# pvjosue/CWFA

Measured on AMD Instinct MI355X. Metric: volumes/sec inverse-pass @512×512×96 fp32; NLL match vs ref (1/2/4/8 GPU), higher is better.
Workload: dtype f32 (storage, accumulation, wavelets, couplings); convolution products on the bf16 matrix cores from an exact three-way bf16 split of both fp32 operands, six products per fp32 product: fp32-equivalent; plain-fp32-MFMA figure: fp32_mfma; 1 GPU; 512x512x96 volume, 4-scale CWFA (CAT blocks, 64 ch) + LRNN inverse, z=0, batch 1/GPU, random-init weights (BASELINE.json configs[2]); precision=split, parallelism=replicated x1 (independent volumes per GPU, no collective)

## Files before the change

cwfa_amd/_lib.py:

```python
import ctypes as C
import os

_HERE = os.path.dirname(os.path.abspath(__file__))
LIB_PATH = os.path.join(_HERE, "libcwfa_hip.so")

CLAMP = {"NONE": 0, "ATAN": 1, "TANH": 2, "SIGMOID": 3}
ACT = {None: 0, "none": 0, "elu": 1, "prelu": 2, "gelu": 3, "relu": 4}
CHAIN_MAX = 8

c_f32p = C.c_void_p
c_i64p = C.c_void_p
c_f64p = C.c_void_p


class AffineStage(C.Structure):
    _fields_ = [("s_raw", c_f32p), ("t", c_f32p), ("s_bs", C.c_int64), ("t_bs", C.c_int64), ("clamp_kind", C.c_int),
                ("clamp", C.c_float), ("pre_scale", C.c_float), ("t_neg_div_sqrt2", C.c_int), ("perm", c_i64p),
                ("perm_axis", C.c_int), ("gin", C.c_int)]


class Chain(C.Structure):
    _fields_ = [("n_stages", C.c_int), ("stage", AffineStage * CHAIN_MAX), ("src_c", C.c_void_p), ("src_h", C.c_void_p)]


# ... 53 lines not shown
    "cwfa_haar2d_inv_f32": (i, [p, p, i, i, i, i, i, f, p]),
    "cwfa_haar3d_fwd_f32": (i, [p, p, i, i, i, i, i, f, i64, p]),
    "cwfa_haar3d_inv_f32": (i, [p, p, i, i, i, i, i, f, i64, p]),
    "cwfa_gather_f32": (i, [p, p, p, i, i, i, i, i, i64, i64, p]),
    "cwfa_affine_f32": (i, [p, p, C.POINTER(AffineStage), i, i, i, i, i, i64, i64, p, p, p]),
    "cwfa_channel_affine_f32": (i, [p, p, p, p, i, p, p, i, i, i64, i64, i64, p]),
    "cwfa_chain_inv_f32": (i, [p, p, p, C.POINTER(Chain), i, i, i, i, i64, i64, i64, p, p]),
    "cwfa_chain_fwd_f32": (i, [p, p, p, C.POINTER(Chain), p, i, i, i, i, i64, i64, i64, p, p, p]),
    "cwfa_conv2d_packed_floats": (i64, [i, i, i]),
    "cwfa_conv2d_pack_f32": (i, [p, p, i, i, i, i, p]),
    "cwfa_conv2d_f32": (i, [p, p, p, i, i, i, i, i, i, i64, i64, C.POINTER(ConvOpts), p]),
    "cwfa_subnet_pack1x1_f32": (i, [p, p, p]),
    "cwfa_subnet_layer_tape_f32": (i, [p, p, p, p, p, p, p, i, i, i, i64, i64, i64, p]),
    "cwfa_subnet_layer_f32": (i, [p, p, p, p, p, p, i, i, i, i64, i64, p]),
    "cwfa_conv3d_1k1_f32": (i, [p, p, p, p, p, p, p, i, i, i, i, i, p]),
    "cwfa_conv3d_1k1_split_f32": (i, [p, p, p, p, p, p, p, i, i, i, i, i, p]),
    "cwfa_channel_stats_f32": (i, [p, p, i, i, i64, i64, p]),
    "cwfa_bn_fold_f32": (i, [p, d, p, p, p, p, f, p, i, p, p, i, p]),
    "cwfa_maxpool_f32": (i, [p, p, p, p, p, i, i, i, i, i, i, p]),
    "cwfa_sample_stats_f32": (i, [p, p, i, i64, p]),
    "cwfa_layernorm_apply_f32": (i, [p, p, p, p, f, p, i, i64, p]),
    "cwfa_attention_combine_f32": (i, [p, p, p, p, p, p, p, p, i, i, i64, p]),
    "cwfa_scale_channels_f32": (i, [p, p, p, i, i, i64, p]),
    "cwfa_axpby_f32": (i, [p, p, f, f, p, i64, p]),
    "cwfa_bn_running_update_f32": (i, [p, C.c_double, f, p, p, p, i, p]),
    "cwfa_bn_finish_f32": (i, [p, d, p, p, p, f, i, p, p, f, p, p, f, f, i, p, p, i, i, p]),
    "cwfa_chain_bwd_f32": (i, [p, p, C.POINTER(Chain), C.POINTER(ChainGrads), p, p, i, i, i, i, i64, i64, i64, f, f, i, p, p]),
    "cwfa_affine_bwd_f32": (i, [p, p, C.POINTER(AffineStage), i, i, i, i, i, i64, i64, p, p, p, p, p]),
    "cwfa_chain_inv_bwd_f32": (i, [p, p, C.POINTER(Chain), C.POINTER(ChainGrads), i, i, i, i, i64, i64, f, i, i, p, p, p, p]),
    "cwfa_conv2d_wgrad_workspace_bytes": (i64, [i, i, i, i, i, i]),
    "cwfa_conv2d_wgrad_f32": (i, [p, p, p, p, p, i, i, i, i, i, i, i64, i64, f, p]),
    "cwfa_elu_bwd_f32": (i, [p, p, p, p, i, i64, i64, i64, i64, i64, p]),
    "cwfa_conv3d_hidden_fwd_f32": (i, [p, p, p, p, i, i, i, i, i, p]),
    "cwfa_conv3d_hidden_bwd_f32": (i, [p, p, p, p, p, p, i, i, i, i, i, p]),
    "cwfa_conv3d_input_bwd_f32": (i, [p, p, p, i, i, i, i, i, p]),
    "cwfa_conv3d_wgrad_workspace_bytes": (i64, [i, i, i, i]),
    "cwfa_conv3d_wgrad_f32": (i, [p, p, p, p, p, i, i, i, i, i, i, i, f, p]),
    "cwfa_prelu_bwd_f32": (i, [p, p, p, p, p, i, i64, i64, i64, i64, p]),
    "cwfa_plane_affine_f32": (i, [p, p, p, i, p, p, i, i, i64, i64, i64, i64, p]),
    "cwfa_bn_bwd_stats_f32": (i, [p, p, p, p, i, i, i64, i64, i64, p]),
    "cwfa_bn_act_bwd_f32": (i, [p, p, p, i, p, p, p, p, p, i, i, i64, i64, i64, i64, p]),
    "cwfa_maxpool2_bwd_f32": (i, [p, p, p, p, i, i, i, i, p]),
    "cwfa_gelu_f32": (i, [p, p, p, i64, i, p]),
    "cwfa_layernorm_bwd_f32": (i, [p, p, p, p, p, p, p, p, p, i, i64, p]),
    "cwfa_attention_bwd_f32": (i, [p, p, p, p, p, p, p, p, p, i, i, i64, p]),
    "cwfa_split_workspace_bytes": (i64, [i, i, i64]),
    "cwfa_split_input_f32": (i, [p, p, i, i, i64, i64, p, p, i64, p, i64, p]),
    "cwfa_conv_split_packed_bytes": (i64, [i, i, i]),
    "cwfa_conv_split_pack_f32": (i, [p, p, i, i, i, i, p]),
    "cwfa_conv_split_f32": (i, [p, p, p, i, i, i, i, i, i, i64, C.POINTER(ConvOpts), p]),
    "cwfa_conv3x3_split_packed_bytes": (i64, [i, i]),
    "cwfa_conv3x3_split_pack_f32": (i, [p, p, i, i, p]),
    "cwfa_conv3x3_split_f32": (i, [p, p, p, i, i, i, i, i, i64, i64, C.POINTER(ConvOpts), p]),
    "cwfa_conv7x7_split_packed_bytes": (i64, [i, i]),
    "cwfa_conv7x7_split_pack_f32": (i, [p, p, i, i, p]),
    "cwfa_conv7x7_split_f32": (i, [p, p, p, i, i, i, i, i, i64, i64, C.POINTER(ConvOpts), p]),
    "cwfa_couple_rows": (i, [i, p]),
    "cwfa_conv3x3_split_couple_f32": (i, [p, p, p, i, i, i, i, i64, C.POINTER(Couple), p]),
    "cwfa_subnet_layer_split_packed_bytes": (i64, []),
    "cwfa_subnet_layer_split_pack_f32": (i, [p, p, p, p]),
    "cwfa_subnet_layer_split_f32": (i, [p, p, p, p, p, i, i, i, i64, i64, i, p]),
    "cwfa_subnet_layer_split_tape_f32": (i, [p, p, p, p, p, p, i, i, i, i64, i64, i64, p]),
    "cwfa_subnet_layer_first_packed_bytes": (i64, []),
    "cwfa_subnet_layer_first_pack_f32": (i, [p, p, p, i, p, p]),
    "cwfa_subnet_layer_first_f32": (i, [p, p, p, p, p, p, i, i, i, i, i64, i64, i64, i, p]),
    "cwfa_extract_views_f32": (i, [p, p, p, i, i, i, i, i, i, f, f, i64, p]),
    "cwfa_eval_splits": (i64, [i, i64]),
    "cwfa_volume_extrema_f32": (i, [p, p, p, p, i, i64, i64, i64, C.POINTER(EvalAffine), p]),
    "cwfa_volume_metrics_f32": (i, [p, p, p, p, i, i64, i64, i64, C.POINTER(EvalAffine), f, f, f, p]),
    "cwfa_mip3_f32": (i, [p, p, p, p, p, p, i, i, i, i, i64, i64, i, C.POINTER(EvalAffine), C.POINTER(EvalPost), p]),
    "cwfa_projection_compose_f32": (i, [p, p, p, p, p, i, i, i, i, i, i, i, p]),
    "cwfa_roi_means_f32": (i, [p, p, p, i, i, i, i, i, i64, p]),
    "cwfa_select_positive_f32": (i, [p, i, i64, i64, i64, p, p, p, p]),
    "cwfa_prep_volumes_f16": (i, [p, p, p, i, i, i, i, i, i, i, i, i, f, f, i, p]),
    "cwfa_prep_frames_f32": (i, [p, p, i, i, i, i, i, i, i, p]),
    "cwfa_histogram_f32": (i, [p, i64, f, f, p, i, p, i, p]),
    "cwfa_prep_apply_f32": (i, [p, i64, i, f, f, i, p]),
    "cwfa_moments_f64": (i, [p, i64, d, p, p, i, p]),
    "cwfa_stack_mean_std_f32": (i, [p, p, p, i, i64, i64, p]),
    "cwfa_lion_step_f32": (i, [C.POINTER(LionTable), f, f, f, f, p, p, p]),
    "cwfa_wmse_workspace_bytes": (i64, [i64]),
    "cwfa_wmse_loss_f32": (i, [p, p, p, f, f, p, p, p, i64, p]),
}
del i, i64, f, d, p

_lib = None


class CwfaHipError(RuntimeError):
    pass


def lib():
    global _lib
    if _lib is None:
        if not os.path.exists(LIB_PATH):
            raise CwfaHipError(
                f"{LIB_PATH} not found: build the HIP extension first (python -m cwfa_amd.build, or "
                f"__graft_entry__.build()).  cwfa_amd has no CPU / PyTorch fallback.")
        import torch
        h = C.CDLL(LIB_PATH)
        for name, (res, args) in SIGNATURES.items():
            fn = getattr(h, name)
            fn.restype = res
            fn.argtypes = args
        if h.cwfa_version() < 100:
# ... 10 lines not shown
```

cwfa_amd/build.py:

```python
import os
import subprocess
import sys
from concurrent.futures import ThreadPoolExecutor

HERE = os.path.dirname(os.path.abspath(__file__))
CSRC = os.path.join(HERE, "csrc")
INCLUDE = os.path.join(os.path.dirname(HERE), "include")
LIB = os.path.join(HERE, "libcwfa_hip.so")
SOURCES = ["elementwise.hip", "conv2d.hip", "conv_wino.hip", "conv_wino2d.hip", "conv_split_layer.hip", "conv_split3x3.hip", "conv3d.hip", "conv3d_split.hip", "lrnn_ops.hip", "conv_bwd.hip", "eval_ops.hip", "prep_ops.hip", "optim_ops.hip", "loss_ops.hip"]
HIPCC = os.environ.get("HIPCC", "/opt/rocm/bin/hipcc")
FLAGS = ["--offload-arch=gfx950", "-O3", "-fPIC", "-std=c++17", "-ffp-contract=off", "-I", INCLUDE, "-I", CSRC,
         "-Wall", "-Wno-unused-function"]


EXTRA = {"conv3d_split.hip": ["-fno-slp-vectorize"]}


def _newer(src, dst):
    return not os.path.exists(dst) or os.path.getmtime(src) > os.path.getmtime(dst)


def build_all(force=False, verbose=False):
    deps = [os.path.join(CSRC, "common.h"), os.path.join(CSRC, "conv_internal.h"), os.path.join(INCLUDE, "cwfa_hip.h"),
            os.path.abspath(__file__)]
    objs, jobs = [], []
    for s in SOURCES:
        src, obj = os.path.join(CSRC, s), os.path.join(CSRC, s.replace(".hip", ".o"))
        objs.append(obj)
        if force or _newer(src, obj) or any(_newer(d, obj) for d in deps):
            jobs.append([HIPCC, *FLAGS, *EXTRA.get(s, []), "-c", src, "-o", obj])

    def run(cmd):
        if verbose:
            print(" ".join(cmd), flush=True)
        r = subprocess.run(cmd, capture_output=True, text=True)
        if r.returncode != 0:
            raise RuntimeError(f"hipcc failed: {' '.join(cmd)}\n{r.stdout}\n{r.stderr}")
        return r.stderr

    with ThreadPoolExecutor(max_workers=4) as ex:
        for warn in ex.map(run, jobs):
            if verbose and warn.strip():
                print(warn, file=sys.stderr)
    if jobs or force or not os.path.exists(LIB) or any(_newer(o, LIB) for o in objs):
        run([HIPCC, "--offload-arch=gfx950", "-shared", "-fPIC", "-o", LIB, *objs])
    return LIB


if __name__ == "__main__":
    print(build_all(force="--force" in sys.argv, verbose=True))
```

cwfa_amd/ops.py:

```python
import ctypes as C

import torch

from . import _lib
from ._lib import AffineStage, Chain, ConvOpts, check

__all__ = ["haar1d", "haar2d", "gather", "affine", "channel_affine", "chain_inv", "chain_fwd", "pack_conv_weight",
           "conv2d", "conv2d_wgrad", "elu_bwd", "set_precision", "gelu_add", "gelu_bwd", "layernorm_bwd", "attention_bwd", "plane_affine", "bn_bwd_stats", "bn_act_bwd", "maxpool2_bwd", "chain_bwd", "chain_inv_bwd", "prelu_bwd", "conv3d_1k1_backward", "pack_1x1_panel", "pack_split_layer_weight", "subnet_layer", "conv3d_1k1", "channel_stats", "bn_fold", "bn_running_update", "maxpool", "sample_stats", "layernorm_apply",
           "attention_combine", "scale_channels", "axpby", "stage", "lion_step", "global_extrema", "wmse_loss"]


def _stream():
    return C.c_void_p(torch.cuda.current_stream().cuda_stream)


def _p(t):
    return None if t is None else C.c_void_p(t.data_ptr())


def _dev(t, name="tensor"):
    if not torch.is_tensor(t):
        raise TypeError(f"{name}: expected a torch.Tensor, got {type(t)}")
    if not t.is_cuda:
        raise RuntimeError(f"{name}: cwfa_amd runs on MI355X only -- got a {t.device} tensor (no CPU fallback exists)")
# ... 259 lines not shown
            if t is None:
                continue
            t2, bs = planes(t, name)
            if t2.data_ptr() != t.data_ptr() or tuple(t.shape) != (B, Cc, H, W):
                raise ValueError(f"chain backward: {name}[{k}] must be a [B,C,H,W] view with contiguous planes")
            getattr(gr, name)[k] = t.data_ptr()
            getattr(gr, name + "_bs")[k] = bs
    return gr


def chain_inv_bwd(xhat, gt, stages, grads, gscale, loss_kind=2, accumulate=False, want_latent_grad=False, want_low_grad=False):
    L = _lib.lib()
    xhat, xbs = planes(xhat, "xhat")
    gt, gbs = planes(gt, "gt")
    if tuple(xhat.shape) != tuple(gt.shape):
        raise ValueError("chain_inv_bwd: xhat and gt differ in shape")
    B, D, H, W = xhat.shape
    Cc = D // 2
    ch, keep = _chain(stages)
    gr = _chain_grads(grads, (B, Cc, H, W))
    loss = torch.zeros(1, dtype=torch.float64, device=xhat.device)
    if want_low_grad and loss_kind != 0:
        raise ValueError("chain_inv_bwd: dL/dlow is formed from an upstream gradient (loss_kind 0)")
    gz = torch.empty((B, Cc, H, W), dtype=torch.float32, device=xhat.device) if want_latent_grad else None
    glow = torch.empty((B, Cc, H, W), dtype=torch.float32, device=xhat.device) if want_low_grad else None
    check(L.cwfa_chain_inv_bwd_f32(_p(xhat), _p(gt), C.byref(ch), C.byref(gr), B, Cc, H, W, xbs, gbs, float(gscale), int(loss_kind),
                                   int(bool(accumulate)), _p(loss), _p(gz), _p(glow), _stream()), "chain_inv_bwd")
    if want_latent_grad or want_low_grad:
        return loss, gz, glow
    return loss


def chain_bwd(z, stages, grads, final_perm=None, gscale=0.0, ldscale=0.0, gz=None, want_input_grad=False, accumulate=False, gld=None):
    L = _lib.lib()
    z, zbs = planes(z, "z")
    B, Cc, H, W = z.shape
    ch, keep = _chain(stages)
    gr = _chain_grads(grads, (B, Cc, H, W))
    gzbs = 0
    if gz is not None:
        gz, gzbs = planes(gz, "gz")
    gv0 = torch.empty((B, Cc, H, W), dtype=torch.float32, device=z.device) if want_input_grad else None
    if gld is not None:
        gld = _dev(gld, "gld").contiguous()
        if gld.numel() != B:
            raise ValueError("chain_bwd: gld must hold one value per sample")
    check(L.cwfa_chain_bwd_f32(_p(z), _p(gz), C.byref(ch), C.byref(gr), _p(_idx(final_perm)), _p(gv0), B, Cc, H, W, zbs, gzbs,
                               Cc * H * W, float(gscale), float(ldscale), int(bool(accumulate)), _p(gld), _stream()), "chain_bwd")
    return gv0


class PackedConv:
    __slots__ = ("packed", "cout", "cin", "ks", "transposed", "version", "src_ptr", "split", "epoch", "version1", "src_ptr1", "cat_c1",
                 "cat_from", "short")

    def __init__(self, packed, cout, cin, ks, transposed, version, src_ptr, split=False):
        self.packed, self.cout, self.cin, self.ks = packed, cout, cin, ks
        self.transposed, self.version, self.src_ptr = transposed, version, src_ptr
        self.split = split
        self.epoch = _pack_epoch


def pack_conv_weight(w, transposed=False, direct=False):
    L = _lib.lib()
    w = _dev(w, "weight").detach().contiguous()
    if transposed:
        cin, co, kh, kw = w.shape
        if (kh, kw) != (2, 2):
            raise ValueError("only 2x2 stride-2 transposed convolutions are supported")
        cout, ks = 4 * co, 1
    else:
        cout, cin, ks, kw = w.shape
        if ks != kw:
            raise ValueError("square kernels only")
    if direct:
        pass
    elif _split_bf16 and ks == 1 and cout >= 128:
        packed = torch.empty(L.cwfa_conv_split_packed_bytes(cout, cin, ks), dtype=torch.uint8, device=w.device)
        check(L.cwfa_conv_split_pack_f32(_p(w), _p(packed), cout, cin, ks, int(transposed), _stream()), "conv_split_pack")
        return PackedConv(packed, cout, cin, ks, transposed, w._version, w.data_ptr(), split=True)
    narrow_max = 32 if single_product() else SPLIT_3X3_NARROW_MAX
    if not direct and _split_bf16 >= 2 and ks == 3 and cout >= SPLIT_3X3_MIN_COUT and (cout > 32 or (cout <= narrow_max and cin >= 29)):
        packed = torch.empty(L.cwfa_conv3x3_split_packed_bytes(cout, cin), dtype=torch.uint8, device=w.device)
        check(L.cwfa_conv3x3_split_pack_f32(_p(w), _p(packed), cout, cin, _stream()), "conv3x3_split_pack")
        return PackedConv(packed, cout, cin, ks, transposed, w._version, w.data_ptr(), split=True)
    if not direct and SPLIT_7X7 and _split_bf16 >= 2 and ks == 7 and cout <= 64 and cin >= 32:
        packed = torch.empty(L.cwfa_conv7x7_split_packed_bytes(cout, cin), dtype=torch.uint8, device=w.device)
        check(L.cwfa_conv7x7_split_pack_f32(_p(w), _p(packed), cout, cin, _stream()), "conv7x7_split_pack")
        return PackedConv(packed, cout, cin, ks, transposed, w._version, w.data_ptr(), split=True)
    n = L.cwfa_conv2d_packed_floats(cout, cin, ks)
    if n <= 0:
        raise ValueError(f"unsupported filter bank {tuple(w.shape)}")
    packed = torch.empty(n, dtype=torch.float32, device=w.device)
    check(L.cwfa_conv2d_pack_f32(_p(w), _p(packed), cout, cin, ks, int(transposed), _stream()), "conv2d_pack")
    return PackedConv(packed, cout, cin, ks, transposed, w._version, w.data_ptr())


def pack_conv_weight_cat(w, c1):
    w = _dev(w, "weight").detach()
    cout, cin, ks, kw = w.shape
    if ks != 1 or kw != 1 or cout > 64 or not (0 < c1 < cin):
        raise ValueError(f"pack_conv_weight_cat: a 1x1 bank with <= 64 outputs and 0 < c1 < Cin is needed, got {tuple(w.shape)}, c1 = {c1}")
    start = (c1 + 15) // 16 * 16
    wz = torch.zeros((cout, start + cin - c1, 1, 1), dtype=torch.float32, device=w.device)
    wz[:, :c1] = w[:, :c1]
    wz[:, start:] = w[:, c1:]
    pc = pack_conv_weight(wz)
    pc.version, pc.src_ptr = w._version, w.data_ptr()
    pc.cat_c1, pc.cat_from = c1, start
    return pc


def conv_writes_stats(pc, act=None, residual=None, act2=None, out_blocked=False, in_add=False):
    return bool(pc.split and pc.ks == 3 and act in (None, "prelu") and residual is None and act2 is None and not out_blocked
                and not (in_add and act is None))


def conv2d(x, pc, bias=None, act=None, prelu_alpha=None, residual=None, act2=None, in_scale=None, in_shift=None,
           in_add=None, out=None, in_blocked=False, out_blocked=False, cat=None, out_stats=None):
    L = _lib.lib()
    x, xbs = planes(x, "x")
    B, Cin, H, W = x.shape
    o = ConvOpts()
    keep = [x]
    if cat is not None:
        cat, cbs = planes(cat, "cat")
        c1 = getattr(pc, "cat_c1", None)
        if c1 is None or Cin != c1 or tuple(cat.shape) != (B, pc.cin - pc.cat_from, H, W) or in_scale is not None or in_add is not None:
            raise ValueError("conv2d: `cat` needs a bank from pack_conv_weight_cat for exactly these two inputs, and no load-side prologue")
        o.in_cat, o.in_cat_bs, o.in_cat_from, o.in_cat_c1 = cat.data_ptr(), cbs, pc.cat_from, c1
        keep.append(cat)
        Cin = pc.cin
    if Cin != pc.cin:
        raise ValueError(f"conv2d: input has {Cin} channels, filter bank expects {pc.cin}")
    up = bool(pc.transposed)
    oshape = (B, pc.cout // 4, 2 * H, 2 * W) if up else (B, pc.cout, H, W)
    if out is None:
        out = torch.empty(oshape, dtype=torch.float32, device=x.device)
        ybs = oshape[1] * oshape[2] * oshape[3]
    else:
        if tuple(out.shape) != oshape:
            raise ValueError(f"conv2d: out has shape {tuple(out.shape)}, expected {oshape}")
        out_c, ybs = planes(out, "out")
        if out_c.data_ptr() != out.data_ptr():
            raise ValueError("conv2d: `out` must have contiguous planes")
    if bias is not None:
        o.bias = _dev(bias, "bias").data_ptr()
    o.act, o.act2 = _lib.ACT[act], _lib.ACT[act2]
# ... 23 lines not shown
            raise ValueError("conv2d: in_add shape mismatch")
        o.in_add, o.in_add_bs = in_add.data_ptr(), abs_
        keep.append(in_add)
    o.upshuffle2 = int(up)
    if in_blocked:
        if not (pc.split and pc.ks == 3):
            raise ValueError("conv2d: channel-blocked input is read by the split-bf16 3x3 kernel only")
        o.in_blocked8 = 1
    if out_blocked:
        ok3 = (pc.split and pc.ks == 3 and pc.cout % 8 == 0 and residual is None and act2 is None and act in (None, "prelu")
               and not split3x3_narrow(pc.cout) and not (in_add is not None and act is None))
        ok1 = not pc.split and pc.ks == 1 and pc.cout >= 33 and pc.cout % 8 == 0 and not up
        if not (ok3 or ok1):
            raise ValueError("conv2d: channel-blocked output is written by the split-bf16 3x3 kernel (bias / PReLU) and by the "
                             "direct 1x1 kernel with 40..64 output channels only")
        o.out_blocked8 = 1
    if out_stats is not None:
        if not conv_writes_stats(pc, act, residual, act2, out_blocked, in_add is not None):
            raise ValueError("conv2d: out_stats needs the split-bf16 3x3 kernel with an NCHW output and a bias / PReLU epilogue")
        if out_stats.dtype != torch.float64 or out_stats.numel() != 2 * pc.cout or not out_stats.is_cuda:
            raise ValueError("conv2d: out_stats must be a float64 [2*Cout] tensor on the HIP device")
        o.out_stats = out_stats.data_ptr()
    rec = conv_event_sink
    if rec is not None:
        key = (pc.ks, Cin, pc.cout, H, W, B, "%s|%s|%s|%s|%s" % ("pro" if (in_scale is not None or in_add is not None) else "",
                                                                 act or "", "res" if residual is not None else "", act2 or "",
                                                                 ("up" if up else "") + ("+split" if pc.split else "")),
               in_add is not None)
        if rec.want(key):
            e0, e1 = torch.cuda.Event(enable_timing=True), torch.cuda.Event(enable_timing=True)
            e0.record()
    if pc.split and pc.ks == 7:
        if act or act2 or residual is not None or in_scale is not None or in_add is not None:
            raise ValueError("conv2d: the split-bf16 7x7 kernel has a bias-only epilogue and no load-side prologue")
        check(L.cwfa_conv7x7_split_f32(_p(x), _p(pc.packed), _p(out), B, Cin, H, W, pc.cout, xbs, ybs, C.byref(o), _stream()),
              "conv7x7_split")
    elif pc.split and pc.ks == 3:
        if split3x3_narrow(pc.cout) and (in_scale is not None or in_add is not None):
            if (H * W) % 4 == 0:
                x = plane_affine(x, in_scale, in_shift, add=in_add)
            else:
                if in_scale is not None:
                    if in_scale.numel() == Cin:
                        x = channel_affine(x, in_scale.reshape(-1), in_shift.reshape(-1))
                    else:
                        x = torch.cat([channel_affine(x[i:i + 1], in_scale.reshape(B, Cin)[i].contiguous(), in_shift.reshape(B, Cin)[i].contiguous())
                                       for i in range(B)], 0)
                if in_add is not None:
                    x = axpby(x.contiguous(), 1.0, in_add, 1.0)
            x, xbs = planes(x, "x")
            o.in_scale = o.in_shift = o.in_add = None
        check(L.cwfa_conv3x3_split_f32(_p(x), _p(pc.packed), _p(out), B, Cin, H, W, pc.cout, xbs, ybs, C.byref(o),
                                       _stream()), "conv3x3_split")
    elif pc.split:
        ws = torch.empty(L.cwfa_split_workspace_bytes(B, Cin, H * W), dtype=torch.uint8, device=x.device)
        per_sample = in_scale is not None and in_scale.numel() == B * Cin and B > 1
        check(L.cwfa_split_input_f32(_p(x), _p(ws), B, Cin, H * W, xbs, _p(in_scale), _p(in_shift), Cin if per_sample else 0,
                                     _p(in_add), in_add.stride(0) if in_add is not None else 0, _stream()), "split_input")
        o.in_scale = o.in_shift = o.in_add = None
        check(L.cwfa_conv_split_f32(_p(ws), _p(pc.packed), _p(out), B, Cin, H, W, pc.cout, pc.ks, ybs, C.byref(o), _stream()),
              "conv_split")
    else:
        check(L.cwfa_conv2d_f32(_p(x), _p(pc.packed), _p(out), B, Cin, H, W, pc.cout, pc.ks, xbs, ybs, C.byref(o),
                                _stream()), "conv2d")
    if rec is not None and rec.want(key):
        e1.record()
        rec.add(key, e0, e1)
    return out


def pack_couple_weight(w, bias):
    L = _lib.lib()
    w = _dev(w, "weight").detach()
    n2, cin, ks, kw = w.shape
    if ks != 3 or kw != 3 or n2 % 2 or n2 // 2 > 64:
        raise ValueError(f"pack_couple_weight: a [2n,Cin,3,3] bank with n <= 64 is needed, got {tuple(w.shape)}")
    n = n2 // 2
    total = L.cwfa_couple_rows(n, None)
    rows_c = (C.c_int * total)()
    L.cwfa_couple_rows(n, rows_c)
    rows = torch.tensor(list(rows_c), dtype=torch.int64, device=w.device)
    live = (rows >= 0)
    wr = torch.zeros((total, cin, 3, 3), dtype=torch.float32, device=w.device)
    wr[live] = w[rows[live]]
    br = torch.zeros(total, dtype=torch.float32, device=w.device)
    if bias is not None:
        br[live] = _dev(bias, "bias").detach()[rows[live]]
    packed = torch.empty(L.cwfa_conv3x3_split_packed_bytes(total, cin), dtype=torch.uint8, device=w.device)
    check(L.cwfa_conv3x3_split_pack_f32(_p(wr), _p(packed), total, cin, _stream()), "conv3x3_split_pack (coupling bank)")
    pc = PackedConv(packed, n2, cin, 3, False, w._version, w.data_ptr(), split=True)
    pc.version1, pc.src_ptr1 = (bias._version, bias.data_ptr()) if bias is not None else (None, None)
    return pc, br


def conv3x3_couple(u, pc_bias, x, out, clamp_kind, clamp, pre_scale, rev, logdet=None, in_blocked=False):
    L = _lib.lib()
    pc, br = pc_bias
    u, ubs = planes(u, "u")
    B, Cin, H, W = u.shape
    n = pc.cout // 2
    if Cin != pc.cin:
        raise ValueError(f"conv3x3_couple: input has {Cin} channels, filter bank expects {pc.cin}")
    x2, xbs = planes(x, "x")
    o2, obs = planes(out, "out")
    if tuple(x.shape) != (B, n, H, W) or tuple(out.shape) != (B, n, H, W) or o2.data_ptr() != out.data_ptr():
        raise ValueError("conv3x3_couple: x / out must be [B,n,H,W] views with contiguous planes")
# ... 566 lines not shown
    x = _dev(x, "x").contiguous()
    z = None if z is None else _dev(z).contiguous()
    if z is not None and z.numel() != x.numel():
        raise ValueError("axpby: x and z differ in size")
    out = torch.empty_like(x)
    check(L.cwfa_axpby_f32(_p(x), _p(z), float(a), float(b), _p(out), x.numel(), _stream()), "axpby")
    return out


def extract_views(image, coords_yx, subimage_shape, mean=0.0, std=1.0):
    L = _lib.lib()
    image = _dev(image, "image")
    if image.dim() != 4 or image.shape[1] != 1:
        raise ValueError(f"extract_views: image must be [B,1,H,W], got {tuple(image.shape)}")
    if image.dtype != torch.float32:
        raise TypeError("extract_views: fp32 images only")
    image = image if image[0].is_contiguous() else image.contiguous()
    B, _, Hs, Ws = image.shape
    co = torch.as_tensor(coords_yx, dtype=torch.int32).reshape(-1, 2)
    sh, sw = int(subimage_shape[0]), int(subimage_shape[1])
    ys, xs = co[:, 0], co[:, 1]
    if len(co) and (bool(((torch.minimum(ys + sh // 2, torch.tensor(Hs)) - torch.clamp(ys - sh // 2, min=0)) <= 0).any()) or
                    bool(((torch.minimum(xs + sw // 2, torch.tensor(Ws)) - torch.clamp(xs - sw // 2, min=0)) <= 0).any())):
        raise ValueError("extract_views: a lenslet window lies outside the image")
    cod = co.contiguous().to(image.device)
    out = torch.empty((B, len(co), sh, sw), dtype=torch.float32, device=image.device)
    check(L.cwfa_extract_views_f32(_p(image), _p(cod), _p(out), B, Hs, Ws, len(co), sh, sw, float(mean), float(std),
                                   image.stride(0), _stream()), "extract_views")
    return out


_split_bf16 = 0
_precision = "fp32"
_pack_epoch = 0


def single_product():
    return _precision in ("bf16", "fp16")


def pack_epoch():
    return _pack_epoch


def invalidate_packs():
    global _pack_epoch
    _pack_epoch += 1


WINOGRAD_2D_DEFAULT = 512


def set_option(name, value):
    global _split_bf16, _pack_epoch
    _pack_epoch += 1
    if name == "split_bf16":
        _split_bf16 = int(value)
        return
    check(_lib.lib().cwfa_set_option(name.encode(), int(value)), "set_option")


PRECISIONS = ("fp32", "split_bf16", "bf16", "fp16")


def set_precision(mode):
    if mode not in PRECISIONS:
        raise ValueError(f"set_precision: unknown mode {mode!r}")
    global _precision
    _precision = mode
    set_option("split_operand", 0)
    set_option("split_products", 1 if single_product() else 6)
    if mode == "fp16":
        set_option("split_operand", 1)
    set_option("split_bf16", 0 if mode == "fp32" else 2)
    set_option("wgrad_split", 0 if mode == "fp32" else 1)


def copy_channels(src, dst):
    L = _lib.lib()
    s_, sbs = planes(src, "src")
    d_, dbs = planes(dst, "dst")
    if d_.data_ptr() != dst.data_ptr() or tuple(src.shape) != tuple(dst.shape):
        raise ValueError("copy_channels: dst must be a [B,c,H,W] view with contiguous planes of src's shape")
    B, Cc, H, W = s_.shape
    check(L.cwfa_channel_affine_f32(_p(s_), _p(dst), None, None, 0, None, None, B, Cc, H * W, sbs, dbs, _stream()), "copy_channels")
    return dst


def concat_channels(parts):
    L = _lib.lib()
    parts = [planes(t, "part") for t in parts]
    B, _, H, W = parts[0][0].shape
    Ct = sum(t.shape[1] for t, _ in parts)
    out = torch.empty((B, Ct, H, W), dtype=torch.float32, device=parts[0][0].device)
    c0 = 0
    for t, bs in parts:
        if t.shape[0] != B or t.shape[2:] != (H, W):
            raise ValueError("concat_channels: shape mismatch")
        check(L.cwfa_channel_affine_f32(_p(t), C.c_void_p(out.data_ptr() + 4 * c0 * H * W), None, None, 0, None, None, B,
                                        t.shape[1], H * W, bs, Ct * H * W, _stream()), "concat_channels")
        c0 += t.shape[1]
    return out


def eval_affine(step, mean, std):
    a = _lib.EvalAffine()
    a.enabled, a.scale = 1, 2.0 ** -int(step)
    a.std = float(torch.as_tensor(std, dtype=torch.float32).reshape(()).cpu())
# ... 295 lines not shown
```

include/cwfa_hip.h:

```cpp
#ifndef CWFA_HIP_H
#define CWFA_HIP_H

#include <stdint.h>

#ifdef __cplusplus
extern "C" {
#endif

#define CWFA_VERSION 100

enum {
    CWFA_OK = 0,
    CWFA_E_INVAL = -1,
    CWFA_E_SHAPE = -2,
    CWFA_E_ALIGN = -3,
    CWFA_E_HIP = -4
};

enum { CWFA_CLAMP_NONE = 0, CWFA_CLAMP_ATAN = 1, CWFA_CLAMP_TANH = 2, CWFA_CLAMP_SIGMOID = 3 };

enum { CWFA_ACT_NONE = 0, CWFA_ACT_ELU = 1, CWFA_ACT_PRELU = 2, CWFA_ACT_GELU = 3, CWFA_ACT_RELU = 4 };

int cwfa_version(void);
const char* cwfa_last_error(void);
// ... 80 lines not shown
    int64_t in_cat_bs;
    int in_cat_from, in_cat_c1;
    double* out_stats;
    int prelu_per_channel;
} cwfa_conv_opts;

int cwfa_conv2d_f32(const float* x, const float* w_packed, float* y, int B, int Cin, int H, int W, int Cout, int ks,
                    int64_t x_bs, int64_t y_bs, const cwfa_conv_opts* opts, void* stream);

int cwfa_subnet_pack1x1_f32(const float* w, float* panel, void* stream);
int cwfa_subnet_layer_f32(const float* x, const float* w3_packed, const float* b3, const float* w1_panel, const float* b1,
                          float* y, int B, int H, int W, int64_t x_bs, int64_t y_bs, void* stream);
int cwfa_subnet_layer_tape_f32(const float* x, const float* w3_packed, const float* b3, const float* w1_panel, const float* b1,
                               float* y, float* hidden, int B, int H, int W, int64_t x_bs, int64_t y_bs, int64_t hidden_bs,
                               void* stream);

int cwfa_conv3d_1k1_f32(const float* x, const float* w1, const float* b1, const float* alpha, const float* w2,
                        const float* b2, float* y, int B, int D, int H, int W, int K, void* stream);
int cwfa_conv3d_1k1_split_f32(const float* x, const float* w1, const float* b1, const float* alpha, const float* w2,
                              const float* b2, float* y, int B, int D, int H, int W, int K, void* stream);


int cwfa_channel_stats_f32(const float* x, double* stats, int B, int C, int64_t HW, int64_t x_bs, void* stream);
int cwfa_bn_fold_f32(const double* stats, double count, const float* running_mean, const float* running_var,
                     const float* weight, const float* bias, float eps, const float* mask_bc, int B, float* scale,
                     float* shift, int C, void* stream);
int cwfa_bn_finish_f32(double* stats, double count, float* running_mean, float* running_var, long long* num_batches_tracked,
                       float momentum, int update_running, const float* weight, const float* bias, float eps, const float* mask_bc,
                       const float* mask_u, float drop_p, float keep_scale, int B, float* scale, float* shift, int C, int zero_stats,
                       void* stream);
int cwfa_bn_running_update_f32(const double* stats, double count, float momentum, float* running_mean, float* running_var,
                               long long* num_batches_tracked, int C, void* stream);
int cwfa_maxpool_f32(const float* x, float* y, float* full, const float* scale, const float* shift, int B, int C,
                     int H, int W, int Ho, int Wo, void* stream);
int cwfa_sample_stats_f32(const float* x, double* stats, int B, int64_t CHW, void* stream);
int cwfa_layernorm_apply_f32(const float* x, const double* stats, const float* w, const float* b, float eps,
                             float* y, int B, int64_t CHW, void* stream);
int cwfa_attention_combine_f32(const float* mean, const float* w1, const float* b1, const float* w2, const float* b2,
                               const float* m, const float* x, float* out, int B, int C, int64_t HW, void* stream);
int cwfa_scale_channels_f32(const float* x, const float* scale_bc, float* y, int B, int C, int64_t HW, void* stream);
int cwfa_axpby_f32(const float* x, const float* z, float a, float b, float* y, int64_t n, void* stream);

int64_t cwfa_split_workspace_bytes(int B, int Cin, int64_t HW);
int cwfa_split_input_f32(const float* x, void* ws, int B, int Cin, int64_t HW, int64_t x_bs, const float* in_scale,
                         const float* in_shift, int64_t in_affine_bs, const float* in_add, int64_t in_add_bs, void* stream);
int64_t cwfa_conv_split_packed_bytes(int Cout, int Cin, int ks);
int cwfa_conv_split_pack_f32(const float* w, void* packed, int Cout, int Cin, int ks, int transposed, void* stream);
int64_t cwfa_conv3x3_split_packed_bytes(int Cout, int Cin);
int cwfa_conv3x3_split_pack_f32(const float* w, void* packed, int Cout, int Cin, void* stream);
int cwfa_conv3x3_split_f32(const float* x, const void* w_packed, float* y, int B, int Cin, int H, int W, int Cout,
                           int64_t x_bs, int64_t y_bs, const cwfa_conv_opts* opts, void* stream);
int cwfa_conv_split_f32(const void* ws, const void* w_packed, float* y, int B, int Cin, int H, int W, int Cout, int ks, int64_t y_bs,
                           const cwfa_conv_opts* opts, void* stream);
int64_t cwfa_conv7x7_split_packed_bytes(int Cout, int Cin);
int cwfa_conv7x7_split_pack_f32(const float* w, void* packed, int Cout, int Cin, void* stream);
int cwfa_conv7x7_split_f32(const float* x, const void* w_packed, float* y, int B, int Cin, int H, int W, int Cout,
                           int64_t x_bs, int64_t y_bs, const cwfa_conv_opts* opts, void* stream);

typedef struct {
    const float* x;
    float* y;
    int64_t x_bs, y_bs;
    int n;
    int clamp_kind;
    float clamp, pre_scale;
    int rev;
    double* logdet;
    int in_blocked8;
} cwfa_couple;
int cwfa_couple_rows(int n, int* rows);
int cwfa_conv3x3_split_couple_f32(const float* x, const void* w_packed, const float* bias_rows, int B, int Cin, int H, int W,
                                  int64_t x_bs, const cwfa_couple* cp, void* stream);

int64_t cwfa_subnet_layer_split_packed_bytes(void);
int cwfa_subnet_layer_split_pack_f32(const float* w3, const float* w1, void* packed, void* stream);
int cwfa_subnet_layer_split_f32(const float* x, const void* packed, const float* b3, const float* b1, float* y, int B, int H,
                                int W, int64_t x_bs, int64_t y_bs, int layout, void* stream);
int64_t cwfa_subnet_layer_first_packed_bytes(void);
int cwfa_subnet_layer_first_pack_f32(const float* w3c, const float* w1, const float* w0c, int short_form, void* packed, void* stream);
int cwfa_subnet_layer_first_f32(const float* u, const float* x, const void* packed, const float* b3, const float* b1, float* y, int B,
                                int u_ch, int H, int W, int64_t u_bs, int64_t x_bs, int64_t y_bs, int layout, void* stream);
int cwfa_subnet_layer_split_tape_f32(const float* x, const void* packed, const float* b3, const float* b1, float* y, float* hid, int B,
                                     int H, int W, int64_t x_bs, int64_t y_bs, int64_t hid_bs, void* stream);

int cwfa_extract_views_f32(const float* image, const int* coords_yx, float* views, int B, int Hs, int Ws, int nviews, int sh,
                           int sw, float mean, float stdv, int64_t image_bs, void* stream);


typedef struct {
    float* ds[CWFA_CHAIN_MAX];
    float* dt[CWFA_CHAIN_MAX];
    int64_t ds_bs[CWFA_CHAIN_MAX], dt_bs[CWFA_CHAIN_MAX];
} cwfa_chain_grads;

int cwfa_chain_bwd_f32(const float* z, const float* gz, const cwfa_chain* ch, const cwfa_chain_grads* grads,
                       const int64_t* final_perm, float* gv0, int B, int C, int H, int W, int64_t z_bs, int64_t gz_bs,
                       int64_t gv0_bs, float gscale, float ldscale, int accumulate, const float* gld, void* stream);

int cwfa_chain_inv_bwd_f32(const float* xhat, const float* gt, const cwfa_chain* ch, const cwfa_chain_grads* grads, int B, int C,
                           int H, int W, int64_t xhat_bs, int64_t gt_bs, float gscale, int loss_kind, int accumulate,
                           double* loss_sum, float* gz_out, float* glow_out, void* stream);

int cwfa_affine_bwd_f32(const float* x, const float* g, const cwfa_affine_stage* st, int rev, int B, int C, int H, int W,
                        int64_t x_bs, int64_t g_bs, const float* gld, float* gx, float* gs_raw, float* gt_raw, void* stream);

int64_t cwfa_conv2d_wgrad_workspace_bytes(int B, int Cin, int H, int W, int Cout, int ks);
// ... 97 lines not shown
```

Before: 53.49 volumes/s.

## Add fused split-bf16 transposed 1x1 upsample conv kernel with pixel-shuffle epilogue

Adds a dedicated kernel for the transposed 1x1 (2x upsampling) split-bf16 conv. It splits the fp32 input into bf16 parts inside the kernel, double-buffering input and weight slices in LDS with async weight DMA, and writes the 2x2 upsampled output directly with a DPP lane swap for wide stores. This avoids the separate input-split workspace pass and its round trip through global memory. It needs an extra packed weight copy, applies only when there is no add, residual or activation and the shapes qualify, and is gated by a new option that defaults to on.

```diff
diff --git a/cwfa_amd/_lib.py b/cwfa_amd/_lib.py
--- a/cwfa_amd/_lib.py
+++ b/cwfa_amd/_lib.py
@@ -129,6 +129,9 @@
     "cwfa_conv3x3_split_packed_bytes": (i64, [i, i]),
     "cwfa_conv3x3_split_pack_f32": (i, [p, p, i, i, p]),
     "cwfa_conv3x3_split_f32": (i, [p, p, p, i, i, i, i, i, i64, i64, C.POINTER(ConvOpts), p]),
+    "cwfa_conv_up_split_packed_bytes": (i64, [i, i]),
+    "cwfa_conv_up_split_pack_f32": (i, [p, p, i, i, p]),
+    "cwfa_conv_up_split_f32": (i, [p, p, p, i, i, i, i, i, i64, i64, C.POINTER(ConvOpts), p]),
     "cwfa_conv7x7_split_packed_bytes": (i64, [i, i]),
     "cwfa_conv7x7_split_pack_f32": (i, [p, p, i, i, p]),
     "cwfa_conv7x7_split_f32": (i, [p, p, p, i, i, i, i, i, i64, i64, C.POINTER(ConvOpts), p]),
diff --git a/cwfa_amd/build.py b/cwfa_amd/build.py
--- a/cwfa_amd/build.py
+++ b/cwfa_amd/build.py
@@ -7,7 +7,7 @@
 CSRC = os.path.join(HERE, "csrc")
 INCLUDE = os.path.join(os.path.dirname(HERE), "include")
 LIB = os.path.join(HERE, "libcwfa_hip.so")
-SOURCES = ["elementwise.hip", "conv2d.hip", "conv_wino.hip", "conv_wino2d.hip", "conv_split_layer.hip", "conv_split3x3.hip", "conv3d.hip", "conv3d_split.hip", "lrnn_ops.hip", "conv_bwd.hip", "eval_ops.hip", "prep_ops.hip", "optim_ops.hip", "loss_ops.hip"]
+SOURCES = ["elementwise.hip", "conv2d.hip", "conv_wino.hip", "conv_wino2d.hip", "conv_split_layer.hip", "conv_split3x3.hip", "conv_up_split.hip", "conv3d.hip", "conv3d_split.hip", "lrnn_ops.hip", "conv_bwd.hip", "eval_ops.hip", "prep_ops.hip", "optim_ops.hip", "loss_ops.hip"]
 HIPCC = os.environ.get("HIPCC", "/opt/rocm/bin/hipcc")
 FLAGS = ["--offload-arch=gfx950", "-O3", "-fPIC", "-std=c++17", "-ffp-contract=off", "-I", INCLUDE, "-I", CSRC,
          "-Wall", "-Wno-unused-function"]
diff --git a/cwfa_amd/csrc/conv_up_split.hip b/cwfa_amd/csrc/conv_up_split.hip
--- /dev/null
+++ b/cwfa_amd/csrc/conv_up_split.hip
@@ -0,0 +1,318 @@
+#include "conv_internal.h"
+
+extern int g_cwfa_split_xcd_map;
+
+namespace {
+
+typedef unsigned u32x2 __attribute__((ext_vector_type(2)));
+
+constexpr int CT = 256, TP = 128;
+constexpr int XPB = 4 * TP * 16;
+constexpr int XB = 3 * XPB;
+constexpr int WSL = 3 * 4 * CT * 16;
+constexpr int OFF_W = 2 * XB;
+constexpr int LDS_BYTES = OFF_W + 2 * WSL;
+static_assert(LDS_BYTES <= 160 * 1024, "LDS budget");
+
+struct UParams {
+    const float* x;
+    const void* wp;
+    float* y;
+    const float* bias;
+    const float* in_scale;
+    const float* in_shift;
+    int in_affine_bs;
+    int B, Cin, H, W, Cout, nsteps, ntiles, ctiles, xcd_map;
+    int wide;
+    int64_t x_bs, y_bs;
+};
+
+template <bool SIX, bool F16 = false>
+__global__ __launch_bounds__(512, 1) void conv_up_split_kernel(UParams p) {
+    extern __shared__ __attribute__((aligned(16))) char lds[];
+    const int tid = threadIdx.x, lane = tid & 63, c16 = lane & 15, g = lane >> 4;
+    const int wave = __builtin_amdgcn_readfirstlane(tid >> 6);
+    const int wm = wave & 3, wn = wave >> 2;
+    const int HW = p.H * p.W;
+    const int plane = HW * 4;
+    constexpr unsigned OOB = 0x80000000u;
+    constexpr int NQ = SIX ? 3 : 1;
+    const int b = blockIdx.z;
+    int sp, ct;
+    if (p.xcd_map && (p.ntiles & 7) == 0) {
+        const int xcd = blockIdx.x & 7, slot = blockIdx.x >> 3;
+        sp = xcd * (p.ntiles >> 3) + slot / p.ctiles;
+        ct = slot % p.ctiles;
+    } else {
+        sp = blockIdx.x / p.ctiles;
+        ct = blockIdx.x % p.ctiles;
+    }
+    const int px0 = sp * TP;
+
+    const int kg = wave >> 1, epx = tid & (TP - 1);
+    const bool fok = px0 + epx < HW;
+    const unsigned fo = fok ? (unsigned)((px0 + epx) * 4) : OOB;
+    const auto rx = CWFA_RSRC(p.x + (int64_t)b * p.x_bs, p.Cin * plane);
+    const bool has_aff = p.in_scale != nullptr;
+    typedef const float __attribute__((address_space(4))) cfloat;
+    cfloat* sc = has_aff ? (cfloat*)(p.in_scale + (int64_t)b * p.in_affine_bs) : nullptr;
+    cfloat* sh = has_aff ? (cfloat*)(p.in_shift + (int64_t)b * p.in_affine_bs) : nullptr;
+    char* const edst = lds + (kg * TP + epx) * 16;
+
+    auto load_entry = [&](float (&xv)[8], int step) {
+        const int ch0 = step * 32 + kg * 8;
+#pragma unroll
+        for (int j = 0; j < 8; ++j) xv[j] = __builtin_bit_cast(float, __builtin_amdgcn_raw_buffer_load_b32(rx, fo, (ch0 + j) * plane, 0));
+    };
+    auto store_entry = [&](const float (&xv)[8], int step, int buf) {
+        const int ch0 = step * 32 + kg * 8;
+        float scv[8], shv[8];
+        if (has_aff) {
+#pragma unroll
+            for (int j = 0; j < 8; ++j) {
+                const int ch = ch0 + j < p.Cin ? ch0 + j : p.Cin - 1;
+                scv[j] = ch0 + j < p.Cin ? sc[ch] : 0.f;
+                shv[j] = ch0 + j < p.Cin ? sh[ch] : 0.f;
+            }
+        }
+        bf16x8 pc[3];
+#pragma unroll
+        for (int j = 0; j < 8; ++j) {
+            float v = xv[j];
+            if (has_aff) v = fok ? v * scv[j] + shv[j] : 0.f;
+            __bf16 a1, a2 = (__bf16)0.f, a3 = (__bf16)0.f;
+            cwfa_split3<SIX, F16>(v, a1, a2, a3);
+            pc[0][j] = a1; pc[1][j] = a2; pc[2][j] = a3;
+        }
+#pragma unroll
+        for (int q = 0; q < NQ; ++q) *reinterpret_cast<bf16x8*>(edst + buf * XB + q * XPB) = pc[q];
+    };
+
+    constexpr int NPC = (SIX ? WSL : WSL / 3) / 1024;
+    const auto rw = CWFA_RSRC(reinterpret_cast<const char*>(p.wp) + (int64_t)ct * p.nsteps * WSL, p.nsteps * WSL);
+    auto dma_w = [&](int slice, int slot) {
+#pragma unroll
+        for (int i = 0; i < NPC / 8; ++i) {
+            const int piece = i * 8 + wave;
+            __builtin_amdgcn_raw_ptr_buffer_load_lds(rw, (lds_ptr)(lds + OFF_W + slot * WSL + piece * 1024), 16, (unsigned)(lane * 16),
+                                                     slice * WSL + piece * 1024, 0, 0);
+        }
+    };
+    static_assert(NPC % 8 == 0, "slice pieces per wave");
+
+    const int alane = OFF_W + (g * CT + wm * 64 + c16) * 16;
+    const int blane = (g * TP + wn * 64 + c16) * 16;
+
+    f32x4 acc[4][4];
+#pragma unroll
+    for (int mt = 0; mt < 4; ++mt)
+#pragma unroll
+        for (int nt = 0; nt < 4; ++nt) acc[mt][nt] = f32x4{0.f, 0.f, 0.f, 0.f};
+    bf16x8 A[2][3], Bq[4][3];
+    float xs[8];
+
+    auto read_a = [&](int set, int abase, int mt) {
+#pragma unroll
+        for (int q = 0; q < NQ; ++q) A[set][q] = *reinterpret_cast<const bf16x8*>(lds + abase + (q * 4 * CT + mt * 16) * 16);
+    };
+    auto read_b = [&](int nt, int bbase) {
+#pragma unroll
+        for (int q = 0; q < NQ; ++q) Bq[nt][q] = *reinterpret_cast<const bf16x8*>(lds + bbase + q * XPB + nt * 256);
+    };
+    auto mfma6 = [&](f32x4& c, const bf16x8 (&a)[3], const bf16x8 (&bb)[3]) {
+        if constexpr (SIX) {
+            CWFA_MFMA(a[2], bb[0], c);
+            CWFA_MFMA(a[1], bb[1], c);
+            CWFA_MFMA(a[0], bb[2], c);
+            CWFA_MFMA(a[1], bb[0], c);
+            CWFA_MFMA(a[0], bb[1], c);
+        }
+        CWFA_MFMA_OP(F16, a[0], bb[0], c);
+    };
+
+    {
+        float x0[8];
+        load_entry(x0, 0);
+        if (p.nsteps > 1) {
+            load_entry(xs, 1);
+        } else {
+#pragma unroll
+            for (int j = 0; j < 8; ++j) xs[j] = 0.f;
+        }
+        dma_w(0, 0);
+        store_entry(x0, 0, 0);
+    }
+    asm volatile("s_waitcnt vmcnt(0)\n\ts_waitcnt lgkmcnt(0)" ::: "memory");
+    __builtin_amdgcn_s_barrier();
+
+    for (int step = 0; step < p.nsteps; ++step) {
+        const int buf = step & 1;
+        const int abase = alane + buf * WSL, bbase = blane + buf * XB;
+        read_a(0, abase, 0);
+#pragma unroll
+        for (int nt = 0; nt < 4; ++nt) read_b(nt, bbase);
+        CWFA_FENCE();
+        __builtin_amdgcn_s_waitcnt(0x0F70);
+        if (step + 1 < p.nsteps) {
+            dma_w(step + 1, buf ^ 1);
+            CWFA_FENCE();
+            store_entry(xs, step + 1, buf ^ 1);
+        }
+        CWFA_FENCE();
+#pragma unroll
+        for (int mt = 0; mt < 4; ++mt) {
+            if (mt < 3) read_a((mt + 1) & 1, abase, mt + 1);
+            CWFA_FENCE();
+#pragma unroll
+            for (int np = 0; np < 4; np += 2) {
+                mfma6(acc[mt][np], A[mt & 1], Bq[np]);
+                mfma6(acc[mt][np + 1], A[mt & 1], Bq[np + 1]);
+                CWFA_FENCE();
+            }
+            if (mt == 0) {
+                if (step + 2 < p.nsteps) load_entry(xs, step + 2);
+                CWFA_FENCE();
+            }
+        }
+        if (step + 2 < p.nsteps) __builtin_amdgcn_s_waitcnt(0x0078);
+        else __builtin_amdgcn_s_waitcnt(0x0070);
+        __builtin_amdgcn_s_barrier();
+    }
+
+    const auto ry = CWFA_RSRC(p.y + (int64_t)b * p.y_bs, p.Cout * plane);
+    const auto rb = CWFA_RSRC(p.bias ? p.bias : p.y, p.bias ? (p.Cout / 4) * 4 : 0);
+    const int cwave = ct * 64 + wm * 16;
+    unsigned po[4];
+#pragma unroll
+    for (int nt = 0; nt < 4; ++nt) {
+        const int px = px0 + wn * 64 + nt * 16 + c16;
+        const int h = px / p.W, w = px - h * p.W;
+        po[nt] = px < HW ? (unsigned)((4 * h * p.W + 2 * w) * 4) + (unsigned)g * (unsigned)(4 * plane) : OOB;
+    }
+    const bool odd = (c16 & 1) != 0;
+    if (p.wide) {
+#pragma unroll
+        for (int nt = 0; nt < 4; ++nt)
+            if (po[nt] != OOB && odd) po[nt] += (unsigned)(8 * p.W) - 8u;
+    }
+    auto swap_pair = [](float v) {
+        return __builtin_bit_cast(float, __builtin_amdgcn_update_dpp(0, __builtin_bit_cast(int, v), 0xB1, 0xF, 0xF, true));
+    };
+#pragma unroll
+    for (int mt = 0; mt < 4; ++mt) {
+        const float bias = __builtin_bit_cast(float, __builtin_amdgcn_raw_buffer_load_b32(rb, (unsigned)(4 * g), (cwave + mt * 4) * 4, 0));
+        const int soff = (cwave + mt * 4) * 4 * plane;
+#pragma unroll
+        for (int nt = 0; nt < 4; ++nt) {
+            const f32x2 top = {acc[mt][nt][0] + bias, acc[mt][nt][1] + bias}, bot = {acc[mt][nt][2] + bias, acc[mt][nt][3] + bias};
+            if (p.wide) {
+                const float g0 = swap_pair(odd ? top[0] : bot[0]), g1 = swap_pair(odd ? top[1] : bot[1]);
+                const f32x4 o4 = odd ? f32x4{g0, g1, bot[0], bot[1]} : f32x4{top[0], top[1], g0, g1};
+                cwfa_buffer_store_b128(__builtin_bit_cast(u32x4, o4), ry, po[nt], soff);
+                continue;
+            }
+            __builtin_amdgcn_raw_buffer_store_b64(__builtin_bit_cast(u32x2, top), ry, po[nt], soff, 0);
+            __builtin_amdgcn_raw_buffer_store_b64(__builtin_bit_cast(u32x2, bot), ry, po[nt] + (unsigned)(8 * p.W), soff, 0);
+        }
+        CWFA_FENCE();
+    }
+}
+
+template <bool F16 = false>
+__global__ __launch_bounds__(256) void conv_up_pack_kernel(const float* __restrict__ w, uint4* __restrict__ out, int Cout, int Cin, int nsteps,
+                                                           int64_t total) {
+    const int64_t i = (int64_t)blockIdx.x * blockDim.x + threadIdx.x;
+    if (i >= total) return;
+    const int col = (int)(i % CT), g = (int)((i / CT) % 4), s = (int)((i / (4 * CT)) % nsteps), ctile = (int)(i / ((int64_t)4 * CT * nsteps));
+    const int row = ctile * CT + col;
+    unsigned short pc[3][8];
+#pragma unroll
+    for (int j = 0; j < 8; ++j) {
+        const int ci = s * 32 + g * 8 + j;
+        const float v = ci < Cin ? w[(int64_t)ci * Cout + row] : 0.f;
+        __bf16 a1, a2, a3;
+        if constexpr (F16) {
+            cwfa_split3<false, true>(v, a1, a2, a3);
+            a2 = a3 = __builtin_bit_cast(__bf16, (unsigned short)0);
+        } else {
+            cwfa_split3<true>(v, a1, a2, a3);
+        }
+        pc[0][j] = __builtin_bit_cast(unsigned short, a1);
+        pc[1][j] = __builtin_bit_cast(unsigned short, a2);
+        pc[2][j] = __builtin_bit_cast(unsigned short, a3);
+    }
+#pragma unroll
+    for (int q = 0; q < 3; ++q) {
+        uint4 v4;
+        v4.x = pc[q][0] | ((unsigned)pc[q][1] << 16);
+        v4.y = pc[q][2] | ((unsigned)pc[q][3] << 16);
+        v4.z = pc[q][4] | ((unsigned)pc[q][5] << 16);
+        v4.w = pc[q][6] | ((unsigned)pc[q][7] << 16);
+        out[(((int64_t)ctile * nsteps + s) * 3 + q) * 4 * CT + g * CT + col] = v4;
+    }
+}
+
+inline int up_nsteps(int Cin) { return (Cin + 31) / 32; }
+
+}
+
+extern "C" int64_t cwfa_conv_up_split_packed_bytes(int Cout, int Cin) {
+    if (Cout <= 0 || Cout % CT != 0 || Cin <= 0) return -1;
+    return (int64_t)(Cout / CT) * up_nsteps(Cin) * WSL;
+}
+
+extern "C" int cwfa_conv_up_split_pack_f32(const float* w, void* packed, int Cout, int Cin, void* stream) {
+    CWFA_REQUIRE(w && packed, CWFA_E_INVAL, "cwfa_conv_up_split_pack_f32: null pointer");
+    CWFA_REQUIRE(Cout > 0 && Cout % CT == 0 && Cin > 0, CWFA_E_SHAPE,
+                 "cwfa_conv_up_split_pack_f32: the packed rows 4 * Co must be a multiple of 256 (got %d)", Cout);
+    CWFA_REQUIRE(cwfa_aligned16(packed), CWFA_E_ALIGN, "cwfa_conv_up_split_pack_f32: packed image must be 16-byte aligned");
+    const int nsteps = up_nsteps(Cin);
+    const int64_t total = (int64_t)(Cout / CT) * nsteps * 4 * CT;
+    return cwfa_with_operand([&](auto, auto f16) -> int {
+        hipLaunchKernelGGL(conv_up_pack_kernel<f16>, dim3((unsigned)((total + 255) / 256)), dim3(256), 0, (hipStream_t)stream, w,
+                           reinterpret_cast<uint4*>(packed), Cout, Cin, nsteps, total);
+        CWFA_LAUNCH_CHECK("cwfa_conv_up_split_pack_f32");
+        return CWFA_OK;
+    });
+}
+
+extern "C" int cwfa_conv_up_split_f32(const float* x, const void* w_packed, float* y, int B, int Cin, int H, int W, int Cout, int64_t x_bs,
+                                      int64_t y_bs, const cwfa_conv_opts* opts, void* stream) {
+    CWFA_REQUIRE(B >= 0 && Cin > 0 && Cout > 0 && H >= 0 && W >= 0, CWFA_E_INVAL, "cwfa_conv_up_split_f32: bad size");
+    CWFA_REQUIRE(Cout % CT == 0, CWFA_E_SHAPE, "cwfa_conv_up_split_f32: the packed rows 4 * Co must be a multiple of 256 (got %d)", Cout);
+    if (B == 0 || H == 0 || W == 0) return CWFA_OK;
+    CWFA_REQUIRE(x && w_packed && y, CWFA_E_INVAL, "cwfa_conv_up_split_f32: null pointer");
+    CWFA_REQUIRE(cwfa_aligned16(w_packed), CWFA_E_ALIGN, "cwfa_conv_up_split_f32: packed weights must be 16-byte aligned");
+    CWFA_REQUIRE((reinterpret_cast<uintptr_t>(y) & 7u) == 0 && (y_bs & 1) == 0, CWFA_E_ALIGN,
+                 "cwfa_conv_up_split_f32: the output (base and batch stride) must be 8-byte aligned");
+    UParams p{};
+    if (opts) {
+        CWFA_REQUIRE(!opts->in_add && !opts->residual && opts->act == CWFA_ACT_NONE && opts->act2 == CWFA_ACT_NONE && !opts->in_blocked8 &&
+                         !opts->out_blocked8 && !opts->in_cat && !opts->out_stats,
+                     CWFA_E_INVAL, "cwfa_conv_up_split_f32: bias-only epilogue, affine-only prologue, NCHW maps");
+        CWFA_REQUIRE(!opts->in_scale == !opts->in_shift, CWFA_E_INVAL, "cwfa_conv_up_split_f32: in_scale and in_shift go together");
+        p.bias = opts->bias;
+        p.in_scale = opts->in_scale;
+        p.in_shift = opts->in_shift;
+        p.in_affine_bs = opts->in_affine_bs;
+    }
+    p.x = x; p.wp = w_packed; p.y = y;
+    p.B = B; p.Cin = Cin; p.H = H; p.W = W; p.Cout = Cout; p.x_bs = x_bs; p.y_bs = y_bs;
+    p.nsteps = up_nsteps(Cin);
+    const int64_t HW = (int64_t)H * W;
+    CWFA_REQUIRE((Cin + 64) * HW * 4 < (1ll << 31) && (int64_t)Cout * HW * 4 + 16 * (int64_t)W < (1ll << 31) && (int64_t)p.nsteps * WSL < (1ll << 31),
+                 CWFA_E_SHAPE, "cwfa_conv_up_split_f32: one sample's input / output / one cout tile's weights must stay below 2 GiB");
+    p.ntiles = (int)((HW + TP - 1) / TP);
+    p.ctiles = Cout / CT;
+    p.xcd_map = g_cwfa_split_xcd_map;
+    p.wide = (W & 1) == 0 && cwfa_aligned16(y) && (y_bs & 3) == 0;
+    CWFA_REQUIRE((int64_t)p.ntiles * p.ctiles < (1ll << 31) && B <= 65535, CWFA_E_SHAPE, "cwfa_conv_up_split_f32: grid too large");
+    return cwfa_with_operand([&](auto six, auto f16) -> int {
+        constexpr auto kern = &conv_up_split_kernel<six, f16>;
+        const int rc = cwfa_max_lds<kern>(LDS_BYTES, "cwfa_conv_up_split_f32");
+        if (rc) return rc;
+        hipLaunchKernelGGL(kern, dim3((unsigned)(p.ntiles * p.ctiles), 1, B), dim3(512), LDS_BYTES, (hipStream_t)stream, p);
+        CWFA_LAUNCH_CHECK("cwfa_conv_up_split_f32");
+        return CWFA_OK;
+    });
+}
diff --git a/cwfa_amd/ops.py b/cwfa_amd/ops.py
--- a/cwfa_amd/ops.py
+++ b/cwfa_amd/ops.py
@@ -335,13 +335,14 @@
 
 class PackedConv:
     __slots__ = ("packed", "cout", "cin", "ks", "transposed", "version", "src_ptr", "split", "epoch", "version1", "src_ptr1", "cat_c1",
-                 "cat_from", "short")
+                 "cat_from", "short", "packed_up")
 
     def __init__(self, packed, cout, cin, ks, transposed, version, src_ptr, split=False):
         self.packed, self.cout, self.cin, self.ks = packed, cout, cin, ks
         self.transposed, self.version, self.src_ptr = transposed, version, src_ptr
         self.split = split
         self.epoch = _pack_epoch
+        self.packed_up = None
 
 
 def pack_conv_weight(w, transposed=False, direct=False):
@@ -361,7 +362,11 @@
     elif _split_bf16 and ks == 1 and cout >= 128:
         packed = torch.empty(L.cwfa_conv_split_packed_bytes(cout, cin, ks), dtype=torch.uint8, device=w.device)
         check(L.cwfa_conv_split_pack_f32(_p(w), _p(packed), cout, cin, ks, int(transposed), _stream()), "conv_split_pack")
-        return PackedConv(packed, cout, cin, ks, transposed, w._version, w.data_ptr(), split=True)
+        pc = PackedConv(packed, cout, cin, ks, transposed, w._version, w.data_ptr(), split=True)
+        if transposed and up_split_qualifies(cout, cin):
+            pc.packed_up = torch.empty(L.cwfa_conv_up_split_packed_bytes(cout, cin), dtype=torch.uint8, device=w.device)
+            check(L.cwfa_conv_up_split_pack_f32(_p(w), _p(pc.packed_up), cout, cin, _stream()), "conv_up_split_pack")
+        return pc
     narrow_max = 32 if single_product() else SPLIT_3X3_NARROW_MAX
     if not direct and _split_bf16 >= 2 and ks == 3 and cout >= SPLIT_3X3_MIN_COUT and (cout > 32 or (cout <= narrow_max and cin >= 29)):
         packed = torch.empty(L.cwfa_conv3x3_split_packed_bytes(cout, cin), dtype=torch.uint8, device=w.device)
@@ -377,6 +382,13 @@
     packed = torch.empty(n, dtype=torch.float32, device=w.device)
     check(L.cwfa_conv2d_pack_f32(_p(w), _p(packed), cout, cin, ks, int(transposed), _stream()), "conv2d_pack")
     return PackedConv(packed, cout, cin, ks, transposed, w._version, w.data_ptr())
+
+
+UP_SPLIT_FUSED = 1
+
+
+def up_split_qualifies(rows, cin):
+    return rows % 256 == 0 and cin % 32 == 0
 
 
 def pack_conv_weight_cat(w, c1):
@@ -506,6 +518,10 @@
             o.in_scale = o.in_shift = o.in_add = None
         check(L.cwfa_conv3x3_split_f32(_p(x), _p(pc.packed), _p(out), B, Cin, H, W, pc.cout, xbs, ybs, C.byref(o),
                                        _stream()), "conv3x3_split")
+    elif (pc.split and up and UP_SPLIT_FUSED and pc.packed_up is not None and in_add is None and residual is None and not o.act
+          and not o.act2 and out.data_ptr() % 8 == 0 and ybs % 2 == 0):
+        check(L.cwfa_conv_up_split_f32(_p(x), _p(pc.packed_up), _p(out), B, Cin, H, W, pc.cout, xbs, ybs, C.byref(o), _stream()),
+              "conv_up_split")
     elif pc.split:
         ws = torch.empty(L.cwfa_split_workspace_bytes(B, Cin, H * W), dtype=torch.uint8, device=x.device)
         per_sample = in_scale is not None and in_scale.numel() == B * Cin and B > 1
@@ -1178,8 +1194,11 @@
 
 
 def set_option(name, value):
-    global _split_bf16, _pack_epoch
+    global _split_bf16, _pack_epoch, UP_SPLIT_FUSED
     _pack_epoch += 1
+    if name == "up_split_fused":
+        UP_SPLIT_FUSED = int(value)
+        return
     if name == "split_bf16":
         _split_bf16 = int(value)
         return
diff --git a/include/cwfa_hip.h b/include/cwfa_hip.h
--- a/include/cwfa_hip.h
+++ b/include/cwfa_hip.h
@@ -156,6 +156,10 @@
                            int64_t x_bs, int64_t y_bs, const cwfa_conv_opts* opts, void* stream);
 int cwfa_conv_split_f32(const void* ws, const void* w_packed, float* y, int B, int Cin, int H, int W, int Cout, int ks, int64_t y_bs,
                            const cwfa_conv_opts* opts, void* stream);
+int64_t cwfa_conv_up_split_packed_bytes(int Cout, int Cin);
+int cwfa_conv_up_split_pack_f32(const float* w, void* packed, int Cout, int Cin, void* stream);
+int cwfa_conv_up_split_f32(const float* x, const void* w_packed, float* y, int B, int Cin, int H, int W, int Cout, int64_t x_bs,
+                           int64_t y_bs, const cwfa_conv_opts* opts, void* stream);
 int64_t cwfa_conv7x7_split_packed_bytes(int Cout, int Cin);
 int cwfa_conv7x7_split_pack_f32(const float* w, void* packed, int Cout, int Cin, void* stream);
 int cwfa_conv7x7_split_f32(const float* x, const void* w_packed, float* y, int B, int Cin, int H, int W, int Cout,
```

Result: no change. 53.58 volumes/s (median of 6 runs) (+0.2%).
